# yuliangguo/OmniFusion

Measured on AMD Instinct MI355X. Metric: panoramas/sec at 512x1024 ERP, N=18 256^2 patches; equi2pers+pers2equi GB/s vs HBM peak, higher is better.
Workload: dtype f16x3 (fp16 hi/lo pairs, fp32 accumulate: fp32-class); 1 GPU; cfg2/cfg4 shard: 8 panoramas/GPU/step, 512x1024 ERP, fov 80, nrows 4 (18 patches); full single-pass spherical_fusion forward (confidence=True) at patch size 128 — the only size the reference network exists at (SURVEY 0.1); random-init weights (seed 42); inputs resident in HBM; resample pair at 18x256^2 reported in roofline_resample; per_gpu_batch=8, global_batch=8, parallelism=image-sharded x1, execution=3 forwards in flight per GPU on 3 streams (spherical_fusion.pipelined)

## Files before the change

### include/omnifusion.h

```cpp
#ifndef OMNIFUSION_H_
#define OMNIFUSION_H_

#include <stddef.h>
#include <stdint.h>

#ifdef __cplusplus
extern "C" {
#endif

#define OMNI_VERSION 200

enum omni_status {
    OMNI_OK = 0,
    OMNI_ERR_INVALID = 1,
    OMNI_ERR_HIP = 2,
    OMNI_ERR_UNSUPPORTED = 3
};

enum omni_layout { OMNI_LAYOUT_BCHWN = 0, OMNI_LAYOUT_BNCHW = 1, OMNI_LAYOUT_BNHWC = 2,
                   OMNI_LAYOUT_BCHNW = 3  };
enum omni_dtype { OMNI_F32 = 0, OMNI_F16 = 1 };

typedef void* omni_stream_t;
typedef struct omni_geometry omni_geometry_t;
// ... 40 lines not shown

int omni_equi2pers_bwd(const void* grad_pers, void* grad_erp, int dtype, int B, int C, int H, int W,
                       int ph, int pw, int nrows, float fov_h, float fov_w, int layout, omni_stream_t stream);
int omni_pers2equi_bwd(const void* grad_erp, void* grad_pers, int dtype, int B, int C, int ph, int pw,
                       int H, int W, int nrows, float fov_h, float fov_w, int layout, omni_stream_t stream);
int omni_conv2d_nhwc_f32(const float* src1, const float* src2, const float* wt, const float* bias,
                         const float* res, float* dst, int M, int H, int W, int C1, int C2, int Cout,
                         int KH, int KW, int stride, int pad, int act, omni_stream_t stream);
int omni_conv2d_splitk_plan(long long rows, int Cout, int ksteps);
int omni_conv2d_nhwc_f32_ws(const float* src1, const float* src2, const float* wt, const float* bias,
                            const float* res, float* dst, int M, int H, int W, int C1, int C2, int Cout,
                            int KH, int KW, int stride, int pad, int act, int splitk, float* ws, size_t ws_bytes,
                            omni_stream_t stream);
int omni_conv2d_nhwc_f16x3_ws(const float* src1, const float* src2, const void* wt16, const float* bias,
                              const float* res, float* dst, int M, int H, int W, int C1, int C2, int Cout,
                              int KH, int KW, int stride, int pad, int act, int splitk, float* ws, size_t ws_bytes,
                              omni_stream_t stream);
int omni_conv2d_sh_f16x3_ws(const void* src1, const void* src2, const void* wt16, const float* bias,
                            const void* res, void* dst, int fmt, int M, int H, int W, int C1, int C2, int Cout,
                            int KH, int KW, int stride, int pad, int act, int splitk, float* ws, size_t ws_bytes,
                            omni_stream_t stream);
int omni_gemm_rows_sh_f16x3(const void* x, const void* wt16r, const float* bias, const float* res, void* dst, int fmt,
                            int rows, int K, int N, int act, omni_stream_t stream);
int omni_gemm_rows_pack(const void* wt16, void* wt16r, int N, int K, omni_stream_t stream);
int omni_gemm_rows_ln_sh_f16x3(const float* x, const float* ln_weight, const float* ln_bias, float eps, const void* wt16r, const float* bias,
                               const float* res, void* dst, int fmt, int rows, int N, int act, omni_stream_t stream);
int omni_conv3x3_up2_sh_f16x3(const void* src, const void* wt16, const float* bias, void* dst, int fmt,
                              int M, int Hl, int Wl, int C, int Cout, int act, omni_stream_t stream);
size_t omni_up2_heads_scratch_bytes(int M, int P);
int omni_conv3x3_up2_heads_sh_f16x3(const void* src, const void* wt16, const float* bias, const void* heads_w16f, float bias_pred, float bias_weight,
                                    float* scratch, size_t scratch_bytes, float* out_a, float* out_c, int M, int P, int confidence, omni_stream_t stream);
int omni_conv3x3_up2_heads_sh_f16x1(const void* src, const void* wt16, const float* bias, const void* heads_w16f, float bias_pred, float bias_weight,
                                    float* scratch, size_t scratch_bytes, float* out_a, float* out_c, int M, int P, int confidence, omni_stream_t stream);
int omni_heads_pack_f16x3(const float* w_host, void* dst_host);
int omni_conv2d_sh_f16x3_post_ws(const void* src1, const void* src2, const void* wt16, const float* bias,
                                 const void* res, void* dst, int fmt, int M, int H, int W, int C1, int C2, int Cout,
                                 int KH, int KW, int stride, int pad, int act, int splitk, float* ws, size_t ws_bytes,
                                 const float* post, size_t post_elems, omni_stream_t stream);
int omni_wino_input_sh(const void* src, void* V, int M, int H, int W, int C, omni_stream_t stream);
int omni_conv3x3_wino_sh_f16x3(const void* V, const void* wt16, const float* bias, const void* res, void* dst, int fmt,
                               int M, int H, int W, int C, int Cout, int act, int splitk, float* ws, size_t ws_bytes, omni_stream_t stream);
int omni_sh_from_f32(const float* src, void* dst, size_t n, omni_stream_t stream);
int omni_sh_to_f32(const void* src, float* dst, size_t n, omni_stream_t stream);
int omni_sh_overflow(int* flag, int reset);
int omni_stem_f32(const float* src, const float* wt, const float* bias, float* dst, int M, int P, omni_stream_t stream);
int omni_maxpool3x3s2_f32(const float* src, float* dst, int M, int H, int W, int C, omni_stream_t stream);
int omni_upsample_bilinear_f32(const float* src, float* dst, int M, int H, int W, int C, int Ho, int Wo, omni_stream_t stream);
int omni_add_hw_f32(float* x, const float* y, int M, int HW, int C, omni_stream_t stream);
int omni_add_period_f32(float* x, const float* y, size_t total, size_t period, omni_stream_t stream);
int omni_stem_sh(const float* src, const float* wt, const float* bias, void* dst, int M, int P, omni_stream_t stream);
int omni_stem_sh_f16x3(const float* src, const void* wt16, const float* bias, void* dst, int M, int P, omni_stream_t stream);
int omni_stem_sh_f16x1(const float* src, const void* wt16, const float* bias, void* dst, int M, int P, omni_stream_t stream);
int omni_maxpool3x3s2_sh(const void* src, void* dst, int M, int H, int W, int C, omni_stream_t stream);
int omni_upsample_bilinear_sh(const void* src, void* dst, int M, int H, int W, int C, int Ho, int Wo, omni_stream_t stream);
int omni_up2_tapsum_sh(const float* y, const float* bias, void* dst, int M, int Hl, int Wl, int Cout, int act, omni_stream_t stream);
int omni_add_hw_sh(void* x, const float* y, int M, int HW, int C, omni_stream_t stream);
int omni_add_period_sh(void* x, const float* y, size_t total, size_t period, omni_stream_t stream);
int omni_layernorm512_sh(const float* x, const float* g, const float* b, void* y, int rows, float eps, omni_stream_t stream);
int omni_gemm_rows_slices_sh_f16x3(const void* x, const void* wt16r, float* parts, int rows, int K, int N, int slices, omni_stream_t stream);
int omni_gemm_rows_ln_parts_sh_f16x3(const float* parts, int nparts, const float* pbias, const float* pres, float* xout,
                                     const float* ln_weight, const float* ln_bias, float eps, const void* wt16r, const float* bias,
                                     void* dst, int fmt, int rows, int N, int act, omni_stream_t stream);
int omni_splitk_reduce_ln512(const float* parts, int nparts, const float* bias, const float* res, float* tok, const float* ln_weight, const float* ln_bias,
                             float eps, void* y, int fmt, int rows, omni_stream_t stream);
int omni_gemm_sh_f16x3_ln512_ws(const void* x, const void* wt16, const float* bias, const float* res, float* tok, const float* ln_g, const float* ln_b,
                                float eps, void* y, int fmt, int rows, int K, int splitk, float* ws, size_t ws_bytes, omni_stream_t stream);
int omni_attention_qkv_sh(const float* qkv, void* out, int B, int N, omni_stream_t stream);
int omni_token_pack_f32(const float* d, const float* pos, float* tok, int M, int N, int HW, int C, omni_stream_t stream);
int omni_layernorm512_f32(const float* x, const float* g, const float* b, float* y, int rows, float eps, omni_stream_t stream);
int omni_attention_f32(const float* q, const float* kv, float* out, int B, int N, omni_stream_t stream);
int omni_heads_f32(const float* x, const float* w, float bias_pred, float bias_weight, float* out_a, float* out_c,
                   int M, int P, int confidence, omni_stream_t stream);
int omni_mlp_points_f32(const float* xyz, const float* depth, const float* w1, const float* b1, const float* w2,
                        const float* b2, float* out, int Mo, int N, int HW, omni_stream_t stream);

int omni_masked_median_f32(const float* x, const float* mask, size_t n, unsigned* ws, float* out, omni_stream_t stream);
int omni_depth_metrics_f32(float* pred, const float* gt, const float* mask, const float* scale_num, const float* scale_den,
                           size_t n, double* ws, float* out, omni_stream_t stream);

size_t omni_semantic_workspace_bytes(size_t npix);
int omni_semantic_step_f32(const float* logits, const int64_t* target, int B, int C, size_t HW, int64_t ignore_index, int K,
                           void* workspace, float* loss, int64_t* pred, int64_t* confusion, omni_stream_t stream);
int omni_semantic_grad_f32(const float* logits, const int64_t* target, int B, int C, size_t HW, int64_t ignore_index,
                           const void* workspace, const float* grad_out, float* grad_logits, omni_stream_t stream);
int omni_confusion_matrix_i64(const int64_t* pred, const int64_t* gt, size_t n, int K, int64_t* confusion, int64_t* n_bad,
                              omni_stream_t stream);

int omni_preprocess_rgb_u8(const unsigned char* src_hwc, float* dst_chw, int B, int Hs, int Ws, int H, int W, omni_stream_t stream);
int omni_preprocess_depth_u16(const unsigned short* src, float* depth, unsigned char* mask, int B, int Hs, int Ws, int H, int W,
                              float min_depth, float max_depth, omni_stream_t stream);
int omni_png_info(const void* data, size_t nbytes, int* width, int* height, int* bit_depth, int* color_type);
int omni_png_decode(const void* data, size_t nbytes, void* dst, int H, int W, int kind);
int omni_png_decode_batch(const void* const* datas, const size_t* nbytes, void* const* dsts, int n, int H, int W, int kind, int threads);
int omni_zlib_inflate(const void* src, size_t nbytes, void* dst, size_t cap, size_t* produced, size_t* consumed);
int omni_png_checksums(const void* data, size_t nbytes, unsigned* crc32, unsigned* adler32);
size_t omni_berhu_workspace_bytes(int B);
int omni_berhu_loss_f32(const float* pred, const float* gt, const float* mask, const float* weights, int B, size_t per_item,
                        void* workspace, float* loss, omni_stream_t stream);
int omni_berhu_grad_f32(const float* pred, const float* gt, const float* mask, const float* weights, int B, size_t per_item,
                        const void* workspace, const float* grad_out, float* grad_pred, omni_stream_t stream);
int omni_pointcloud_ply_f32(const float* depth, const float* rgb, unsigned char* records, int B, int H, int W, omni_stream_t stream);

size_t omni_dibr_workspace_bytes(int B, int C, int H, int W);
int omni_splat_render_f32(const float* img, const float* depth, const float* coords, float max_depth,
                          float* recon, unsigned char* mask , int B, int C, int H, int W,
                          void* workspace, omni_stream_t stream);
// ... 85 lines not shown
```

### omnifusion_amd/_lib.py

```python
import ctypes
import os

_HERE = os.path.dirname(os.path.abspath(__file__))
LIB_PATH = os.environ.get("OMNI_LIB_VARIANT") or os.path.join(_HERE, "csrc", "libomnifusion_hip.so")
LIB_PATH_DEBUG = os.path.join(_HERE, "csrc", "libomnifusion_hip_dbg.so")

OMNI_OK, OMNI_ERR_INVALID, OMNI_ERR_HIP, OMNI_ERR_UNSUPPORTED = 0, 1, 2, 3
LAYOUT_BCHWN, LAYOUT_BNCHW, LAYOUT_BNHWC, LAYOUT_BCHNW = 0, 1, 2, 3
F32, F16 = 0, 1

_lib = None


class OmniLibraryMissing(ImportError):
    pass


EXPORTS = [
    "omni_version", "omni_last_error", "omni_set_option", "omni_get_option", "omni_num_patches", "omni_patch_centers",
    "omni_geometry_create", "omni_geometry_destroy", "omni_geometry_cache_clear", "omni_geometry_cache_size",
    "omni_equi2pers", "omni_equi2pers_aux", "omni_pers2equi", "omni_pers2equi_conf", "omni_patches_to_planar",
    "omni_equi2pers_g", "omni_pers2equi_g", "omni_equi2pers_bwd", "omni_pers2equi_bwd",
    "omni_conv2d_nhwc_f32", "omni_stem_f32", "omni_maxpool3x3s2_f32", "omni_upsample_bilinear_f32",
    "omni_add_hw_f32", "omni_add_period_f32", "omni_token_pack_f32", "omni_layernorm512_f32",
    "omni_attention_f32", "omni_heads_f32", "omni_mlp_points_f32",
    "omni_conv2d_nhwc_f16x3_ws", "omni_conv2d_sh_f16x3_ws", "omni_conv2d_sh_f16x3_post_ws", "omni_gemm_rows_sh_f16x3", "omni_gemm_rows_ln_sh_f16x3", "omni_gemm_rows_pack", "omni_conv3x3_up2_sh_f16x3", "omni_conv3x3_up2_heads_sh_f16x3", "omni_conv3x3_up2_heads_sh_f16x1", "omni_up2_heads_scratch_bytes", "omni_heads_pack_f16x3", "omni_sh_from_f32", "omni_sh_to_f32", "omni_sh_overflow",
    "omni_stem_sh", "omni_stem_sh_f16x3", "omni_stem_sh_f16x1", "omni_maxpool3x3s2_sh", "omni_upsample_bilinear_sh", "omni_up2_tapsum_sh", "omni_add_hw_sh", "omni_add_period_sh", "omni_layernorm512_sh", "omni_gemm_sh_f16x3_ln512_ws", "omni_gemm_rows_slices_sh_f16x3", "omni_gemm_rows_ln_parts_sh_f16x3", "omni_splitk_reduce_ln512", "omni_wino_input_sh", "omni_conv3x3_wino_sh_f16x3", "omni_attention_qkv_sh",
    "omni_conv2d_splitk_plan", "omni_conv2d_nhwc_f32_ws",
    "omni_masked_median_f32", "omni_depth_metrics_f32",
    "omni_png_info", "omni_png_decode", "omni_png_decode_batch", "omni_zlib_inflate", "omni_png_checksums",
    "omni_preprocess_rgb_u8", "omni_preprocess_depth_u16", "omni_berhu_workspace_bytes", "omni_berhu_loss_f32", "omni_berhu_grad_f32",
    "omni_pointcloud_ply_f32",
    "omni_dibr_workspace_bytes", "omni_splat_render_f32", "omni_dibr_f32",
    "omni_splat_render_wt_f32", "omni_dibr_wt_f32", "omni_dibr_bwd_workspace_bytes", "omni_splat_render_bwd_f32", "omni_dibr_bwd_f32",
    "omni_ssim_f32", "omni_photometric_workspace_bytes", "omni_photometric_grad_scratch_bytes", "omni_photometric_loss_f32",
    "omni_photometric_grad_f32",
    "omni_freeview_rotations", "omni_freeview_equi2pers_f32", "omni_freeview_pers2equi_f32", "omni_freeview_merge_f32",
    "omni_freeview_bwd_workspace_bytes", "omni_freeview_equi2pers_bwd_f32", "omni_freeview_pers2equi_bwd_f32", "omni_freeview_merge_bwd_f32",
    "omni_semantic_workspace_bytes", "omni_semantic_step_f32", "omni_semantic_grad_f32", "omni_confusion_matrix_i64",
    "omni_depth_normals_f32", "omni_sobel_f32", "omni_l1_workspace_bytes", "omni_l1_loss_f32", "omni_l1_grad_f32",
    "omni_geometry_terms_workspace_bytes", "omni_geometry_terms_f32", "omni_geometry_terms_grad_f32",
    "omni_image_diff_f32", "omni_image_diff_norm_f32", "omni_vertex_diff_norm_f32",
    "omni_guided_smoothness_workspace_bytes", "omni_guided_smoothness_f32", "omni_guided_smoothness_grad_f32",
    "omni_depth_smoothness_workspace_bytes", "omni_depth_smoothness_f32", "omni_depth_smoothness_grad_f32",
    "omni_chamfer_workspace_bytes", "omni_chamfer_nn_f32", "omni_chamfer_grad_f32",
]


def load():
    global _lib
    if _lib is not None:
        return _lib
    if not os.path.exists(LIB_PATH):
        raise OmniLibraryMissing(
            f"{LIB_PATH} not found: build it with `python -m omnifusion_amd.build` "
            "(hipcc --offload-arch=gfx950).  There is no fallback path.")
    import torch
    lib = ctypes.CDLL(LIB_PATH)
    lib.omni_last_error.restype = ctypes.c_char_p
    lib.omni_version.restype = ctypes.c_int
    lib.omni_up2_heads_scratch_bytes.restype = ctypes.c_size_t
    lib.omni_dibr_workspace_bytes.restype = ctypes.c_size_t
    lib.omni_splat_render_f32.argtypes = [ctypes.c_void_p] * 3 + [ctypes.c_float] + [ctypes.c_void_p] * 2 + [ctypes.c_int] * 4 + [ctypes.c_void_p] * 2
    lib.omni_dibr_f32.argtypes = [ctypes.c_void_p] * 4 + [ctypes.c_int, ctypes.c_float, ctypes.c_int] + [ctypes.c_void_p] * 2 + \
        [ctypes.c_int] * 4 + [ctypes.c_void_p] * 2
    vp, ci, cf = ctypes.c_void_p, ctypes.c_int, ctypes.c_float
    lib.omni_splat_render_wt_f32.argtypes = [vp] * 3 + [cf] + [vp] * 3 + [ci] * 4 + [vp] * 2
    lib.omni_dibr_wt_f32.argtypes = [vp] * 4 + [ci, cf, ci] + [vp] * 3 + [ci] * 4 + [vp] * 2
    lib.omni_dibr_bwd_workspace_bytes.restype = ctypes.c_size_t
    lib.omni_splat_render_bwd_f32.argtypes = [vp] * 6 + [cf] + [vp] * 3 + [ci] * 4 + [vp] * 2
    lib.omni_dibr_bwd_f32.argtypes = [vp] * 7 + [ci, cf, ci] + [vp] * 2 + [ci] * 4 + [vp] * 2
    lib.omni_ssim_f32.argtypes = [vp] * 2 + [ci] * 5 + [vp, ci, vp, vp]
    lib.omni_photometric_workspace_bytes.restype = ctypes.c_size_t
    lib.omni_photometric_grad_scratch_bytes.restype = ctypes.c_size_t
    lib.omni_photometric_loss_f32.argtypes = [vp, vp, vp, ci, vp, ci] + [ci] * 5 + [vp, ci, cf] + [vp] * 3
    lib.omni_photometric_grad_f32.argtypes = [vp, vp, vp, ci, vp, ci] + [ci] * 5 + [vp, ci, cf] + [vp] * 5
    lib.omni_freeview_rotations.argtypes = [vp, vp, ci, vp, vp]
    lib.omni_freeview_equi2pers_f32.argtypes = [vp] * 3 + [ci] * 7 + [cf, cf, ci, vp]
    lib.omni_freeview_pers2equi_f32.argtypes = [vp] * 4 + [ci] * 6 + [cf, cf, vp]
    lib.omni_freeview_merge_f32.argtypes = [vp] * 4 + [ci] * 7 + [cf, cf, vp]
# ... 94 lines not shown
```

### omnifusion_amd/csrc/omni_net.hip

```cpp
#include <algorithm>
#include "omni_internal.h"
#include "omni_sh.h"

namespace {
typedef float f4v __attribute__((ext_vector_type(4)));

template <bool SH>
__global__ __launch_bounds__(256) void stem_kernel(const float* __restrict__ src, const float* __restrict__ wt,
                                                   const float* __restrict__ bias, void* __restrict__ dst,
                                                   int M, int P, int Po)
{
    __shared__ __attribute__((aligned(16))) float wl[147 * 64];
    __shared__ float in[3][21][22];
    const int t = threadIdx.x;
    const int tiles = Po / 8;
    const int m = blockIdx.x / (tiles * tiles), tt = blockIdx.x % (tiles * tiles);
    const int oy0 = (tt / tiles) * 8, ox0 = (tt % tiles) * 8;
    for (int i = t; i < 147 * 64 / 4; i += 256) reinterpret_cast<f4v*>(wl)[i] = reinterpret_cast<const f4v*>(wt)[i];
    const int iy0 = oy0 * 2 - 3, ix0 = ox0 * 2 - 3;
    for (int i = t; i < 3 * 21 * 21; i += 256) {
        const int c = i / 441, r = (i % 441) / 21, q = i % 21;
        const int iy = iy0 + r, ix = ix0 + q;
        float v = 0.0f;
        if ((unsigned)iy < (unsigned)P && (unsigned)ix < (unsigned)P) v = src[((size_t)m * 3 + c) * P * P + (size_t)iy * P + ix];
// ... 335 lines not shown
            for (int kx = 0; kx < 3; ++kx) {
                const float* px = tile + ((ly + ky) * (HT + 2) + lx + kx) * HPITCH;
                const float* w0 = w + (ky * 3 + kx) * 32; const float* w1 = w0 + 288;
#pragma unroll
                for (int c = 0; c < 32; c += 4) {
                    const f4v v = *reinterpret_cast<const f4v*>(px + c);
                    ap = fmaf(v.x, w0[c], ap); ap = fmaf(v.y, w0[c + 1], ap); ap = fmaf(v.z, w0[c + 2], ap); ap = fmaf(v.w, w0[c + 3], ap);
                    aw = fmaf(v.x, w1[c], aw); aw = fmaf(v.y, w1[c + 1], aw); aw = fmaf(v.z, w1[c + 2], aw); aw = fmaf(v.w, w1[c + 3], aw);
                }
            }
        const int m = tid / (tiles * tiles), tt = tid % (tiles * tiles);
        const int oy = (tt / tiles) * HT + ly, ox = (tt % tiles) * HT + lx;
        if (oy < P && ox < P) {
            const size_t i = ((size_t)m * P + oy) * P + ox;
            const float pr = fmaxf(ap, 0.0f), cf = 1.0f / (1.0f + expf(-aw));
            outa[i] = conf ? pr * cf : pr;
            if (outc) outc[i] = cf;
        }
    }
}

__global__ __launch_bounds__(256) void mlp_points_kernel(const float* __restrict__ xyz, const float* __restrict__ depth,
                                                         const float* __restrict__ w1 , const float* __restrict__ b1,
                                                         const float* __restrict__ w2 , const float* __restrict__ b2,
                                                         float* __restrict__ out, int Mo, int N, int HW)
{
    const int i = blockIdx.x * 256 + threadIdx.x;
    if (i >= Mo * HW) return;
    const int m = i / HW, hw = i % HW, n = m % N;
    const float d = depth ? depth[i] : 1.0f;
    const float x0 = xyz[((size_t)n * 3 + 0) * HW + hw] * d, x1 = xyz[((size_t)n * 3 + 1) * HW + hw] * d, x2 = xyz[((size_t)n * 3 + 2) * HW + hw] * d;
    float hid[16];
#pragma unroll
    for (int j = 0; j < 16; ++j) hid[j] = fmaxf(fmaf(x2, w1[j * 3 + 2], fmaf(x1, w1[j * 3 + 1], fmaf(x0, w1[j * 3], b1[j]))), 0.0f);
    float* o = out + (size_t)i * 64;
    for (int j = 0; j < 64; j += 4) {
        float r[4];
#pragma unroll
        for (int e = 0; e < 4; ++e) {
            float acc = b2[j + e];
#pragma unroll
            for (int k = 0; k < 16; ++k) acc = fmaf(hid[k], w2[(j + e) * 16 + k], acc);
            r[e] = fmaxf(acc, 0.0f);
        }
        f4v v; v.x = r[0]; v.y = r[1]; v.z = r[2]; v.w = r[3];
        *reinterpret_cast<f4v*>(o + j) = v;
    }
}

inline int nblk(size_t n) { return (int)((n + 255) / 256); }
}

#define S_ (hipStream_t)stream
OMNI_SH_OVERFLOW_ACCESSOR(omni_sh_overflow_net)

extern "C" {

int omni_stem_f32(const float* src, const float* wt, const float* bias, float* dst, int M, int P, omni_stream_t stream)
{
    if (P % 16) OMNI_FAIL(OMNI_ERR_INVALID, "omni_stem: patch size must be a multiple of 16");
    const int Po = P / 2;
    hipLaunchKernelGGL(stem_kernel<false>, dim3(M * (Po / 8) * (Po / 8)), dim3(256), 0, S_, src, wt, bias, (void*)dst, M, P, Po);
    OMNI_HIP(hipGetLastError()); return OMNI_OK;
}
int omni_maxpool3x3s2_f32(const float* src, float* dst, int M, int H, int W, int C, omni_stream_t stream)
{
    const int Ho = (H + 2 - 3) / 2 + 1, Wo = (W + 2 - 3) / 2 + 1;
    hipLaunchKernelGGL(maxpool_kernel<false>, dim3(nblk((size_t)M * Ho * Wo * C / 4)), dim3(256), 0, S_, (const void*)src, (void*)dst, M, H, W, C, Ho, Wo);
    OMNI_HIP(hipGetLastError()); return OMNI_OK;
}
int omni_upsample_bilinear_f32(const float* src, float* dst, int M, int H, int W, int C, int Ho, int Wo, omni_stream_t stream)
{
    hipLaunchKernelGGL(upsample_kernel<false>, dim3(nblk((size_t)M * Ho * Wo * C / 4)), dim3(256), 0, S_, (const void*)src, (void*)dst, M, H, W, C, Ho, Wo,
                       (float)H / (float)Ho, (float)W / (float)Wo);
    OMNI_HIP(hipGetLastError()); return OMNI_OK;
}
int omni_add_hw_f32(float* x, const float* y, int M, int HW, int C, omni_stream_t stream)
{
    const size_t total = (size_t)M * HW * C;
    hipLaunchKernelGGL(add_hw_kernel, dim3(nblk(total)), dim3(256), 0, S_, x, y, total, HW, C);
    OMNI_HIP(hipGetLastError()); return OMNI_OK;
}
int omni_add_period_f32(float* x, const float* y, size_t total, size_t period, omni_stream_t stream)
{
    hipLaunchKernelGGL(add_period_kernel, dim3(nblk(total)), dim3(256), 0, S_, x, y, total, period);
    OMNI_HIP(hipGetLastError()); return OMNI_OK;
}
int omni_stem_sh(const float* src, const float* wt, const float* bias, void* dst, int M, int P, omni_stream_t stream)
{
    if (P % 16) OMNI_FAIL(OMNI_ERR_INVALID, "omni_stem: patch size must be a multiple of 16");
    const int Po = P / 2;
    hipLaunchKernelGGL(stem_kernel<true>, dim3(M * (Po / 8) * (Po / 8)), dim3(256), 0, S_, src, wt, bias, dst, M, P, Po);
    OMNI_HIP(hipGetLastError()); return OMNI_OK;
}
int omni_maxpool3x3s2_sh(const void* src, void* dst, int M, int H, int W, int C, omni_stream_t stream)
{
    if (C % 32) OMNI_FAIL(OMNI_ERR_INVALID, "SH tensors need C % 32 == 0");
    const int Ho = (H + 2 - 3) / 2 + 1, Wo = (W + 2 - 3) / 2 + 1;
    hipLaunchKernelGGL(maxpool_kernel<true>, dim3(nblk((size_t)M * Ho * Wo * C / 4)), dim3(256), 0, S_, src, dst, M, H, W, C, Ho, Wo);
    OMNI_HIP(hipGetLastError()); return OMNI_OK;
}
int omni_upsample_bilinear_sh(const void* src, void* dst, int M, int H, int W, int C, int Ho, int Wo, omni_stream_t stream)
{
    if (C % 32) OMNI_FAIL(OMNI_ERR_INVALID, "SH tensors need C % 32 == 0");
    hipLaunchKernelGGL(upsample_sh8_kernel, dim3(nblk((size_t)M * Ho * Wo * C / 8)), dim3(256), 0, S_, (const unsigned char*)src,
                       (unsigned char*)dst, M, H, W, C, Ho, Wo, (float)H / (float)Ho, (float)W / (float)Wo);
    OMNI_HIP(hipGetLastError()); return OMNI_OK;
// ... 78 lines not shown
```

### omnifusion_amd/isa.py

```python
import os
import re
import subprocess
import sys
import tempfile

LLVM = os.environ.get("OMNI_LLVM_BIN", "/opt/rocm/lib/llvm/bin")
TARGET = "hipv4-amdgcn-amd-amdhsa--gfx950"
FORBIDDEN = re.compile(r"\bv_pk_(mul|add|fma)_f32\b")
COUNTED = ("e2p_box_kernel", "p2e_lds_kernel", "p2e_walk_kernel", "e2p_ref_kernel")
HOT = ("conv_sh_kernel", "conv3x3_halo_sh_kernel", "conv3x3_up2_g1_kernel", "stem_f16x3_pc_kernel", "heads_kernel", "maxpool_kernel",
       "layernorm512_kernel", "attention_kernel", "upsample_sh8_kernel")
HOST_ONLY = ("omni_png.o", "omni_geometry.o")


def _device_object(obj, tmp):
    fat = os.path.join(tmp, "fat.bin")
    co = os.path.join(tmp, "dev.co")
    r = subprocess.run([os.path.join(LLVM, "llvm-objcopy"), "--dump-section", f".hip_fatbin={fat}", obj, os.path.join(tmp, "copy.o")],
                       stderr=subprocess.DEVNULL)
    if r.returncode != 0 or not os.path.exists(fat) or os.path.getsize(fat) == 0:
        return None
    subprocess.check_call([os.path.join(LLVM, "clang-offload-bundler"), "--unbundle", "--type=o", f"--input={fat}",
                           f"--targets={TARGET}", f"--output={co}"])
    return co


def disassemble(obj):
    with tempfile.TemporaryDirectory() as tmp:
        co = _device_object(obj, tmp)
        if co is None:
            return ""
        return subprocess.check_output([os.path.join(LLVM, "llvm-objdump"), "-d", "--mcpu=gfx950", co]).decode()


def kernel_meta(obj):
    with tempfile.TemporaryDirectory() as tmp:
        co = _device_object(obj, tmp)
        if co is None:
            return []
        txt = subprocess.check_output([os.path.join(LLVM, "llvm-readelf"), "--notes", co]).decode()
    out, cur = [], None
    keys = {".vgpr_count": "vgpr", ".agpr_count": "agpr", ".sgpr_count": "sgpr", ".group_segment_fixed_size": "lds",
            ".private_segment_fixed_size": "scratch", ".vgpr_spill_count": "vgpr_spill", ".sgpr_spill_count": "sgpr_spill",
            ".name": "name"}
    for line in txt.splitlines():
        m = re.match(r"^  - \.(\w+):\s*(\S+)\s*$", line)
        if m:
            cur = {}
            out.append(cur)
            line = "    ." + m.group(1) + ": " + m.group(2)
        m = re.match(r"^    (\.\w+):\s*(\S+)\s*$", line)
        if m and cur is not None and m.group(1) in keys:
            v = m.group(2)
            cur[keys[m.group(1)]] = v if m.group(1) == ".name" else int(v)
    return [k for k in out if "name" in k]


def demangle(names):
    try:
        p = subprocess.run([os.path.join(LLVM, "llvm-cxxfilt")], input="\n".join(names).encode(), stdout=subprocess.PIPE, check=True)
        return p.stdout.decode().splitlines()
    except Exception:
        return list(names)
# ... 69 lines not shown
```

### omnifusion_amd/model/_engine.py

```python
import ctypes
import os

import torch

from .. import _lib
from ..equi_pers.equi2pers_v3 import equi2pers_patches, equi2pers_aux, pair, _NPATCH
from ..equi_pers.pers2equi_v3 import pers2equi, pers2equi_conf

ACT_NONE, ACT_RELU, ACT_GELU = 0, 1, 2
_LAYERS = [("layer1", 3, 1), ("layer2", 4, 2), ("layer3", 6, 2), ("layer4", 3, 2)]
_BN_EPS = 1e-5
PRECISIONS = ("f16x3", "f16x1", "fp32")


def _p(t):
    return ctypes.c_void_p(t.data_ptr()) if t is not None else None


def split_weights_f16x3(w):
    w = w.to(torch.float32)
    wmax = float(w.abs().max()) if w.numel() else 0.0
    if not wmax < 65504.0:
        raise ValueError(f"folded weight magnitude {wmax:g} is outside the fp16 range of the f16x3 operand format: "
                         "run this checkpoint with OMNI_NET_PRECISION=fp32")
# ... 314 lines not shown
        pending = None
        for i in range(6):
            t = f"t{i}."
            if sh:
                if pending is not None:
                    tok, qkv = self._ln_gemm_parts(pending, t + "norm1.weight", t + "norm1.bias", 1e-5, t + "attn.qkv.w16", M, 1536)
                    pending = None
                elif normed is not None:
                    qkv = self._gemm_sh(normed, t + "attn.qkv.w16", None, M, 512, 1536)
                else:
                    qkv = self._ln_gemm_sh(tok, t + "norm1.weight", t + "norm1.bias", 1e-5, t + "attn.qkv.w16", None, M, 1536)
                att = new(M, 512)
                _lib.check(lib.omni_attention_qkv_sh(_p(qkv), _p(att), bs, N, self._s), "attention")
                tok = self._gemm_sh(att, t + "attn.proj.w16", t + "attn.proj.bias", M, 512, 512, res=tok)
                h = self._ln_gemm_sh(tok, t + "norm2.weight", t + "norm2.bias", 1e-5, t + "mlp.fc1.w16", t + "mlp.fc1.bias", M, 2048, act=ACT_GELU, out_sh=True)
                nxt = (f"t{i + 1}.norm1.weight", f"t{i + 1}.norm1.bias", 1e-5, True) if i < 5 else ("enc_norm.w", "enc_norm.b", 1e-6, False)
                tok, normed, pending = self._fc2_ln(h, t + "mlp.fc2.w16", t + "mlp.fc2.bias", M, tok, nxt)
                continue
            y = self._ln(tok, t + "norm1.weight", t + "norm1.bias", M, 1e-5)
            q = self._gemm(y, t + "attn.q.weight", None, M, 512, 512)
            kv = self._gemm(y, t + "attn.kv.weight", None, M, 512, 1024)
            att = new(M, 512)
            _lib.check(lib.omni_attention_f32(_p(q), _p(kv), _p(att), bs, N, self._s), "attention")
            tok = self._gemm(att, t + "attn.proj.weight", t + "attn.proj.bias", M, 512, 512, res=tok)
            y = self._ln(tok, t + "norm2.weight", t + "norm2.bias", M, 1e-5)
            h = self._gemm(y, t + "mlp.fc1.weight", t + "mlp.fc1.bias", M, 512, 2048, act=ACT_GELU)
            tok = self._gemm(h, t + "mlp.fc2.weight", t + "mlp.fc2.bias", M, 2048, 512, res=tok)
        if sh and pending is not None:
            parts, S, bkey, res_tok = pending
            tok_sum, tok = new(M, 512), new(M, 512)
            _lib.check(lib.omni_splitk_reduce_ln512(_p(parts), S, _p(self.w[bkey]), _p(res_tok), _p(tok_sum), _p(self.w["enc_norm.w"]), _p(self.w["enc_norm.b"]),
                                                    ctypes.c_float(1e-6), _p(tok), 0, M, self._s), "reduce+ln")
        else:
            tok = normed if (sh and normed is not None) else self._ln(tok, "enc_norm.w", "enc_norm.b", M, 1e-6)
        return tok

    def network(self, patches, point_feat, bs, confidence, out=None):
        lib = _lib.load()
        dev = patches.device
        self._s = ctypes.c_void_p(torch.cuda.current_stream(dev).cuda_stream)
        N, P = self.npatches, self.patch_size[0]
        M = bs * N
        self._bs = bs
        P2, P4, P8, P16, P32 = P // 2, P // 4, P // 8, P // 16, P // 32
        new = lambda *s: torch.empty(s, dtype=torch.float32, device=dev)
        conv1 = new(M, P2, P2, 64)
        sh = self.sh
        x = new(M, P4, P4, 64)
        pat = patches.view(M, 3, P, P)
        for m0, m1 in self._chunks(bs, N, self.front_chunk):
            Mc = m1 - m0
            if self.terms == 1 and P % 32:
                raise ValueError(f"precision f16x1 needs a patch size that is a multiple of 32 (got {P})")
            if sh and P % 32 == 0:
                _lib.check((lib.omni_stem_sh_f16x1 if self._x1 else lib.omni_stem_sh_f16x3)(_p(pat[m0:m1]), _p(self.w["stem.w16"]), _p(self.w["stem.b"]), _p(conv1[m0:m1]), Mc, P, self._s), "stem")
            else:
                _lib.check((lib.omni_stem_sh if sh else lib.omni_stem_f32)(_p(pat[m0:m1]), _p(self.w["stem.w"]), _p(self.w["stem.b"]),
                                                                            _p(conv1[m0:m1]), Mc, P, self._s), "stem")
            _lib.check((lib.omni_maxpool3x3s2_sh if sh else lib.omni_maxpool3x3s2_f32)(_p(conv1[m0:m1]), _p(x[m0:m1]), Mc, P2, P2, 64, self._s), "maxpool")
        feats = {}
        cin, size = 64, P4
        for lname, nblk, stride in _LAYERS:
            cout = {"layer1": 64, "layer2": 128, "layer3": 256, "layer4": 512}[lname]
            for i in range(nblk):
                p = f"{lname}.{i}"
                s = stride if i == 0 else 1
                ident = x
                if (p + ".ds.w") in self.w:
                    ident = self._conv(x, p + ".ds", M, size, size, cin, cout, 1, s, 0, ACT_NONE)
                y = self._conv(x, p + ".c1", M, size, size, cin, cout, 3, s, 1, ACT_RELU)
                size = (size + 2 - 3) // s + 1
                fold = sh and self.fold_point_feat and lname == "layer1" and i == nblk - 1
                x = self._conv(y, p + ".c2", M, size, size, cout, cout, 3, 1, 1, ACT_RELU, res=ident, post=point_feat if fold else None)
                cin = cout
            if lname == "layer1" and not (sh and self.fold_point_feat):
                _lib.check((lib.omni_add_period_sh if sh else lib.omni_add_period_f32)(
                    _p(x), _p(point_feat), ctypes.c_size_t(x.numel()), ctypes.c_size_t(point_feat.numel()), self._s), "add point_feat")
            feats[lname] = x
        layer1, layer2, layer3, layer4 = (feats[k] for k in ("layer1", "layer2", "layer3", "layer4"))
        if 32 * P32 * P32 != 512:
            raise RuntimeError(f"patch size {P}: token dim {32 * P32 * P32} != 512 — the reference network only exists at "
                               "patch size 128 (SURVEY.md finding 0.1)")
        d = self._conv(layer4, "down", M, P32, P32, 512, 32, 1, 1, 0, ACT_NONE, out_f32=True)
        tok = self.transformer(d, bs)
        _lib.check((lib.omni_add_hw_sh if sh else lib.omni_add_hw_f32)(_p(layer4), _p(tok), M, P32 * P32, 512, self._s), "token bias")
        x = self._up_conv_taps(layer4, "de_conv0_0", M, P32, P32, 512, 256, ACT_RELU)
        x = self._conv(x, "de_conv0_1", M, P16, P16, 256, 128, 3, 1, 1, ACT_RELU, x2=layer3, C2=256)
        x = self._up_conv_taps(x, "de_conv1_0", M, P16, P16, 128, 128, ACT_RELU)
        x = self._conv(x, "de_conv1_1", M, P8, P8, 128, 64, 3, 1, 1, ACT_RELU, x2=layer2, C2=128)
        x = self._up_conv(x, "de_conv2_0", M, P8, P8, 64, 64, ACT_RELU)
        x = self._conv(x, "de_conv2_1", M, P4, P4, 64, 64, 3, 1, 1, ACT_RELU, x2=layer1, C2=64)
        a, c = out if out is not None else (new(bs, N, 1, P, P), new(bs, N, 1, P, P) if confidence else None)
        av, cv = a.view(M, P, P), c.view(M, P, P) if c is not None else None
        fused = sh and self.fuse_heads and P % 32 == 0
        x_in, de4 = x, (None if fused else new(M, P, P, 32))
        for m0, m1 in self._chunks(bs, N, self.tail_chunk):
            Mc = m1 - m0
            x = self._up_conv(x_in[m0:m1], "de_conv3_0", Mc, P4, P4, 64, 64, ACT_RELU)
            x = self._conv(x, "de_conv3_1", Mc, P2, P2, 64, 32, 3, 1, 1, ACT_RELU, x2=conv1[m0:m1], C2=64)
            if fused:
                nb = int(lib.omni_up2_heads_scratch_bytes(Mc, P))
                hs = new((nb + 3) // 4)
                _lib.check((lib.omni_conv3x3_up2_heads_sh_f16x1 if self._x1 else lib.omni_conv3x3_up2_heads_sh_f16x3)(_p(x), _p(self.w["de_conv4_0.w16"]), _p(self.w["de_conv4_0.b"]), _p(self.w["heads.w16f"]),
                                                               ctypes.c_float(self.head_bias[0]), ctypes.c_float(self.head_bias[1]), _p(hs), ctypes.c_size_t(nb),
                                                               _p(av[m0:m1]), _p(cv[m0:m1]) if cv is not None else None, Mc, P, 1 if confidence else 0, self._s), "up+conv+heads")
                continue
            self._up_conv(x, "de_conv4_0", Mc, P2, P2, 32, 32, ACT_RELU, out_f32=True, out=de4[m0:m1])
            _lib.check(lib.omni_heads_f32(_p(de4[m0:m1]), _p(self.w["heads.w"]), ctypes.c_float(self.head_bias[0]), ctypes.c_float(self.head_bias[1]),
                                          _p(av[m0:m1]), _p(cv[m0:m1]) if cv is not None else None, Mc, P, 1 if confidence else 0, self._s), "heads")
        self.last = {"de_conv4_0": de4, "layer4": layer4}
        return a, c

    fuse_heads = os.environ.get("OMNI_FUSE_HEADS", "1") != "0"

    tail_chunk = 0
    front_chunk = 0

    @staticmethod
    def _chunks(bs, N, per):
        per = bs if per <= 0 else min(per, bs)
        return [(b0 * N, min(bs, b0 + per) * N) for b0 in range(0, bs, per)]

    def blend(self, a, c, erp_hw):
        P = self.patch_size
        if c is not None:
            return pers2equi_conf(a, c, self.fov, self.nrows, P, erp_hw, layout=_lib.LAYOUT_BNCHW)
        return pers2equi(a, self.fov, self.nrows, P, erp_hw, None, layout=_lib.LAYOUT_BNCHW)

    def mlp_points(self, name, xyz, depth, Mo):
        lib = _lib.load()
        P4 = self.patch_size[0] // 4
        out = torch.empty((Mo, P4, P4, 64), dtype=torch.float32, device=xyz.device)
        s = ctypes.c_void_p(torch.cuda.current_stream(xyz.device).cuda_stream)
        _lib.check(lib.omni_mlp_points_f32(_p(xyz), _p(depth), _p(self.w[name + ".w1"]), _p(self.w[name + ".b1"]),
                                           _p(self.w[name + ".w2"]), _p(self.w[name + ".b2"]), _p(out), Mo, self.npatches,
                                           P4 * P4, s), "mlp_points")
        return out

    def check_input(self, rgb):
        if not isinstance(rgb, torch.Tensor) or rgb.dim() != 4 or rgb.shape[1] != 3:
            raise ValueError("expected an RGB panorama batch [B,3,H,W]")
        if not rgb.is_cuda:
            raise ValueError("the model runs on an MI355X only (got a CPU tensor); there is no CPU path")
        if rgb.dtype != torch.float32:
            raise ValueError("float32 input expected")
        if _NPATCH[self.nrows] != self.npatches:
            raise ValueError("npatches does not match nrows")
```

Before: 4149 panoramas/s.

## Fuse ResNet stem conv with 3x3 stride-2 maxpool in one warp-specialized kernel

Adds a kernel that computes the 7x7 stride-2 stem conv on an output tile plus a one-pixel halo using MFMA f16x3. It keeps the tile in LDS and applies the 3x3/s2 maxpool there, writing both conv1 and the pooled output. Producer waves prefetch and split the input image into double-buffered LDS while consumer waves compute, which hides load latency. This removes the separate maxpool launch and its reread of conv1 from HBM. The cost is recomputing halo pixels per tile and a complex kernel with high LDS use, which may limit occupancy.

```diff
diff --git a/include/omnifusion.h b/include/omnifusion.h
--- a/include/omnifusion.h
+++ b/include/omnifusion.h
@@ -116,6 +116,7 @@
 int omni_stem_sh_f16x3(const float* src, const void* wt16, const float* bias, void* dst, int M, int P, omni_stream_t stream);
 int omni_stem_sh_f16x1(const float* src, const void* wt16, const float* bias, void* dst, int M, int P, omni_stream_t stream);
 int omni_maxpool3x3s2_sh(const void* src, void* dst, int M, int H, int W, int C, omni_stream_t stream);
+int omni_stem_pool_sh_f16x3(const float* src, const void* wt16, const float* bias, void* conv1, void* pooled, int M, int P, omni_stream_t stream);
 int omni_upsample_bilinear_sh(const void* src, void* dst, int M, int H, int W, int C, int Ho, int Wo, omni_stream_t stream);
 int omni_up2_tapsum_sh(const float* y, const float* bias, void* dst, int M, int Hl, int Wl, int Cout, int act, omni_stream_t stream);
 int omni_add_hw_sh(void* x, const float* y, int M, int HW, int C, omni_stream_t stream);
diff --git a/omnifusion_amd/_lib.py b/omnifusion_amd/_lib.py
--- a/omnifusion_amd/_lib.py
+++ b/omnifusion_amd/_lib.py
@@ -25,7 +25,7 @@
     "omni_add_hw_f32", "omni_add_period_f32", "omni_token_pack_f32", "omni_layernorm512_f32",
     "omni_attention_f32", "omni_heads_f32", "omni_mlp_points_f32",
     "omni_conv2d_nhwc_f16x3_ws", "omni_conv2d_sh_f16x3_ws", "omni_conv2d_sh_f16x3_post_ws", "omni_gemm_rows_sh_f16x3", "omni_gemm_rows_ln_sh_f16x3", "omni_gemm_rows_pack", "omni_conv3x3_up2_sh_f16x3", "omni_conv3x3_up2_heads_sh_f16x3", "omni_conv3x3_up2_heads_sh_f16x1", "omni_up2_heads_scratch_bytes", "omni_heads_pack_f16x3", "omni_sh_from_f32", "omni_sh_to_f32", "omni_sh_overflow",
-    "omni_stem_sh", "omni_stem_sh_f16x3", "omni_stem_sh_f16x1", "omni_maxpool3x3s2_sh", "omni_upsample_bilinear_sh", "omni_up2_tapsum_sh", "omni_add_hw_sh", "omni_add_period_sh", "omni_layernorm512_sh", "omni_gemm_sh_f16x3_ln512_ws", "omni_gemm_rows_slices_sh_f16x3", "omni_gemm_rows_ln_parts_sh_f16x3", "omni_splitk_reduce_ln512", "omni_wino_input_sh", "omni_conv3x3_wino_sh_f16x3", "omni_attention_qkv_sh",
+    "omni_stem_sh", "omni_stem_sh_f16x3", "omni_stem_sh_f16x1", "omni_maxpool3x3s2_sh", "omni_stem_pool_sh_f16x3", "omni_upsample_bilinear_sh", "omni_up2_tapsum_sh", "omni_add_hw_sh", "omni_add_period_sh", "omni_layernorm512_sh", "omni_gemm_sh_f16x3_ln512_ws", "omni_gemm_rows_slices_sh_f16x3", "omni_gemm_rows_ln_parts_sh_f16x3", "omni_splitk_reduce_ln512", "omni_wino_input_sh", "omni_conv3x3_wino_sh_f16x3", "omni_attention_qkv_sh",
     "omni_conv2d_splitk_plan", "omni_conv2d_nhwc_f32_ws",
     "omni_masked_median_f32", "omni_depth_metrics_f32",
     "omni_png_info", "omni_png_decode", "omni_png_decode_batch", "omni_zlib_inflate", "omni_png_checksums",
diff --git a/omnifusion_amd/csrc/omni_net.hip b/omnifusion_amd/csrc/omni_net.hip
--- a/omnifusion_amd/csrc/omni_net.hip
+++ b/omnifusion_amd/csrc/omni_net.hip
@@ -411,7 +411,13 @@
 }
 
 #define S_ (hipStream_t)stream
-OMNI_SH_OVERFLOW_ACCESSOR(omni_sh_overflow_net)
+OMNI_SH_OVERFLOW_ACCESSOR(omni_sh_overflow_net_own)
+int omni_sh_overflow_stem_pool(unsigned* out, int reset);
+int omni_sh_overflow_net(unsigned* out, int reset)
+{
+    const int a = omni_sh_overflow_net_own(out, reset), b = omni_sh_overflow_stem_pool(out, reset);
+    return (a != 0 || b != 0) ? -1 : 0;
+}
 
 extern "C" {
 
diff --git a/omnifusion_amd/csrc/omni_stem_pool.hip b/omnifusion_amd/csrc/omni_stem_pool.hip
--- /dev/null
+++ b/omnifusion_amd/csrc/omni_stem_pool.hip
@@ -0,0 +1,252 @@
+#include "omni_conv_sh_common.h"
+
+namespace {
+
+constexpr int SP_TH = 8, SP_TW = 16;
+constexpr int SP_WH = SP_TH + 1, SP_WW = SP_TW + 1, SP_NPIX = SP_WH * SP_WW;
+constexpr int SP_IH = 2 * SP_WH + 5, SP_IW = 2 * SP_WW + 5, SP_IP = 40, SP_IS = 48;
+constexpr int SP_G = 6;
+constexpr int SP_IMG = 3 * SP_IH * SP_IP, SP_IPT = (SP_IMG + 255) / 256, SP_IMGS = 3 * SP_IH * SP_IS;
+constexpr int SP_PITCH = 272;
+constexpr int SP_NBLK = (SP_NPIX + 31) / 32;
+constexpr int SP_CONS = 2 * SP_NBLK;
+constexpr int SP_THREADS = 64 * (SP_CONS + 4);
+constexpr int SP_COPY = SP_TH * SP_TW * 16 / 64;
+constexpr int SP_POOL = (SP_TH / 2) * (SP_TW / 2) * 8 / 64;
+static_assert(SP_IW + 1 <= SP_IP && SP_IP <= SP_IS, "the kx = 7 slot of the last window column reads a parked zero");
+
+__global__ __launch_bounds__(SP_THREADS) void stem_pool_sh_kernel(const float* __restrict__ src, const void* __restrict__ wt16, const float* __restrict__ bias,
+                                                                  void* __restrict__ conv1, void* __restrict__ pooled, int M, int P, int tpb)
+{
+    __shared__ __attribute__((aligned(1024))) unsigned char wl[64 * SP_G * 128];
+    __shared__ __attribute__((aligned(16))) _Float16 imh[2][SP_IMGS], iml[2][SP_IMGS];
+    __shared__ __attribute__((aligned(16))) unsigned char otile[2][SP_NPIX * SP_PITCH];
+    __shared__ __attribute__((aligned(16))) float sbias[64];
+    const int t = threadIdx.x, lane = t & 63;
+    const int wave = __builtin_amdgcn_readfirstlane(t >> 6);
+    const int Po = P / 2, Pq = P / 4;
+    const int sps = Po / SP_TH, tps = Po / SP_TW, ntiles = M * sps * tps;
+    const int T0 = blockIdx.x * tpb, T1 = min(T0 + tpb, ntiles);
+    if (T0 >= T1) return;
+    auto where = [&](int T, int& m, int& oy0, int& ox0) { const int strip = T / tps; ox0 = (T - strip * tps) * SP_TW; m = strip / sps; oy0 = (strip - m * sps) * SP_TH; };
+
+    if (wave >= SP_CONS) {
+        const int ft = t - 64 * SP_CONS;
+        float pre[SP_IPT], nxt[SP_IPT];
+        int po[SP_IPT], rq[SP_IPT], ls[SP_IPT];
+#pragma unroll
+        for (int k = 0; k < SP_IPT; ++k) {
+            const int i = ft + 256 * k;
+            const int c = i / (SP_IH * SP_IP), r = (i % (SP_IH * SP_IP)) / SP_IP, q = i % SP_IP;
+            po[k] = (c * P + r) * P + q;
+            rq[k] = (i < SP_IMG && q < SP_IW) ? (r | (q << 8)) : -1;
+            ls[k] = i < SP_IMG ? (i / SP_IP) * SP_IS + q : -1;
+        }
+        int fm, fs, fc;
+        { const int strip = T0 / tps; fc = T0 - strip * tps; fm = strip / sps; fs = strip - fm * sps; }
+        auto fetch = [&](float (&v)[SP_IPT]) {
+            const int m = fm, oy0 = fs * SP_TH, ox0 = fc * SP_TW;
+            if (++fc == tps) { fc = 0; if (++fs == sps) { fs = 0; ++fm; } }
+            const int iy0 = oy0 * 2 - 5, ix0 = ox0 * 2 - 5;
+            const float* base = src + (size_t)m * 3 * P * P + ((long long)iy0 * P + ix0);
+#pragma unroll
+            for (int k = 0; k < SP_IPT; ++k) {
+                const int iy = iy0 + (rq[k] & 0xff), ix = ix0 + (rq[k] >> 8);
+                v[k] = (rq[k] >= 0 && (unsigned)iy < (unsigned)P && (unsigned)ix < (unsigned)P) ? base[po[k]] : 0.0f;
+            }
+        };
+        auto park = [&](int b, const float (&v)[SP_IPT]) {
+#pragma unroll
+            for (int k = 0; k < SP_IPT; ++k) {
+                const float x = v[k];
+                const _Float16 hh = (fabsf(x) < 6.103515625e-05f) ? (_Float16)0.0f : (_Float16)x;
+                if (ls[k] >= 0) { imh[b][ls[k]] = hh; iml[b][ls[k]] = (_Float16)((x - (float)hh) * 2048.0f); }
+            }
+        };
+        fetch(pre);
+        if (T0 + 1 < T1) fetch(nxt);
+        park(0, pre);
+        if (T0 + 2 < T1) fetch(pre);
+        __syncthreads();
+        int b = 0, T = T0 + 1;
+        for (;;) {
+            if (T >= T1) break;
+            b ^= 1; park(b, nxt);
+            if (T + 2 < T1) fetch(nxt);
+            __syncthreads();
+            if (++T >= T1) break;
+            b ^= 1; park(b, pre);
+            if (T + 2 < T1) fetch(pre);
+            __syncthreads();
+            ++T;
+        }
+        __syncthreads();
+        return;
+    }
+
+    const int blk = wave % SP_NBLK, cj = wave / SP_NBLK;
+    if (wave < 8) {
+        const int pr = wave & 3, ch = wave >> 2;
+        const int gs = (lane & 15) ^ ((4 * pr + (lane >> 4)) & 15);
+        const int rl = 8 * pr + 2 * (lane >> 4) + (gs >> 3), pc16 = (gs & 7) * 16;
+        const rsrc_t rsw = make_rsrc(wt16, (size_t)64 * SP_G * 128);
+#pragma unroll
+        for (int g = 0; g < SP_G; ++g)
+            dma16(rsw, wl + g * 8192 + pr * 1024 + ch * 4096, ((rl + 32 * ch) * SP_G + g) * 128 + pc16, 0);
+    }
+    int fo[4];
+    {
+        const int r = lane & 31, v = r >> 1, h = lane >> 5;
+#pragma unroll
+        for (int k = 0; k < 4; ++k) fo[k] = v * 256 + ((((r & 1) * 8 + 2 * k + h) ^ v) * 16);
+    }
+    const int npix = 32 * blk + (lane & 31);
+    const bool live = npix < SP_NPIX;
+    const int py = (live ? npix : SP_NPIX - 1) / SP_WW, px = (live ? npix : SP_NPIX - 1) % SP_WW;
+    int rowoff[2 * SP_G];
+#pragma unroll
+    for (int f = 0; f < 2 * SP_G; ++f) {
+        int rr = 2 * f + (lane >> 5);
+        rr = rr < 21 ? rr : 20;
+        rowoff[f] = ((rr / 7) * SP_IH + rr % 7 + 2 * py) * SP_IS + 2 * px;
+    }
+    if (wave == 0) sbias[lane] = bias ? bias[lane] : 0.0f;
+    wait_vm<0>();
+    wait_lds_reads();
+    __syncthreads();
+
+    f16v acc, acc1;
+    auto kloop = [&](int b) {
+        const _Float16* ih = imh[b];
+        const _Float16* il = iml[b];
+        acc = (f16v)(0.0f); acc1 = (f16v)(0.0f);
+#pragma unroll
+        for (int g = 0; g < SP_G; ++g)
+#pragma unroll
+            for (int kc = 0; kc < 2; ++kc) {
+                const int ro = rowoff[2 * g + kc];
+                h8v ah, al;
+#pragma unroll
+                for (int u = 0; u < 4; ++u) {
+                    const h2v xh = *reinterpret_cast<const h2v*>(ih + ro + 2 * u);
+                    ah[2 * u] = xh[0]; ah[2 * u + 1] = xh[1];
+                    const h2v xl = *reinterpret_cast<const h2v*>(il + ro + 2 * u);
+                    al[2 * u] = xl[0]; al[2 * u + 1] = xl[1];
+                }
+                const unsigned char* bp = wl + g * 8192 + cj * 4096;
+                const h8v bh = *reinterpret_cast<const h8v*>(bp + fo[kc]);
+                const h8v bl = *reinterpret_cast<const h8v*>(bp + fo[2 + kc]);
+                acc = __builtin_amdgcn_mfma_f32_32x32x16_f16(bh, ah, acc, 0, 0, 0);
+                acc1 = __builtin_amdgcn_mfma_f32_32x32x16_f16(bl, ah, acc1, 0, 0, 0);
+                acc1 = __builtin_amdgcn_mfma_f32_32x32x16_f16(bh, al, acc1, 0, 0, 0);
+            }
+    };
+    auto deposit = [&](int T, int ob) {
+        int m, oy0, ox0;
+        where(T, m, oy0, ox0);
+        const bool inimg = (py > 0 || oy0 > 0) && (px > 0 || ox0 > 0);
+        unsigned char* dp = otile[ob] + npix * SP_PITCH + cj * 128 + 8 * (lane >> 5);
+#pragma unroll
+        for (int q = 0; q < 4; ++q) {
+            f4v v;
+#pragma unroll
+            for (int e = 0; e < 4; ++e) v[e] = acc_join<false>(acc1[4 * q + e], acc[4 * q + e]);
+            v += *reinterpret_cast<const f4v*>(sbias + 32 * cj + 8 * q + 4 * (lane >> 5));
+#pragma unroll
+            for (int e = 0; e < 4; ++e) v[e] = inimg ? fmaxf(v[e], 0.f) : 0.0f;
+            h4v hi, lo;
+            sh_split4(v, hi, lo);
+            if (live) { *reinterpret_cast<h4v*>(dp + 16 * q) = hi; *reinterpret_cast<h4v*>(dp + 16 * q + 64) = lo; }
+        }
+    };
+    const bool pools = (wave & 2) != 0 && wave < 8;
+    static_assert(SP_COPY == 32 && SP_POOL == 4 && SP_CONS == 10, "the task split above is written for these counts");
+    auto out = [&](int T, int ob) {
+        int m, oy0, ox0;
+        where(T, m, oy0, ox0);
+        const unsigned char* tp = otile[ob];
+        auto piece = [&](int task, const unsigned char*& lp, size_t& go) {
+            const int idx = task * 64 + lane, op = idx >> 4, pc = idx & 15;
+            const int oy = op / SP_TW, ox = op % SP_TW;
+            lp = tp + ((oy + 1) * SP_WW + ox + 1) * SP_PITCH + 16 * pc;
+            go = (((size_t)m * Po + oy0 + oy) * Po + ox0 + ox) * 256 + 16 * pc;
+        };
+        {
+            const unsigned char *l0, *l1, *l2; size_t g0, g1, g2;
+            piece(wave, l0, g0); piece(wave + SP_CONS, l1, g1); piece(wave + 2 * SP_CONS, l2, g2);
+            const uint4 v0 = *reinterpret_cast<const uint4*>(l0), v1 = *reinterpret_cast<const uint4*>(l1), v2 = *reinterpret_cast<const uint4*>(l2);
+            *reinterpret_cast<uint4*>((unsigned char*)conv1 + g0) = v0;
+            *reinterpret_cast<uint4*>((unsigned char*)conv1 + g1) = v1;
+            *reinterpret_cast<uint4*>((unsigned char*)conv1 + g2) = v2;
+        }
+        if (wave < SP_COPY - 3 * SP_CONS) {
+            const unsigned char* lp; size_t go;
+            piece(3 * SP_CONS + wave, lp, go);
+            *reinterpret_cast<uint4*>((unsigned char*)conv1 + go) = *reinterpret_cast<const uint4*>(lp);
+        }
+        if (pools) {
+            const int ppy = (wave >> 2) * 2 + (wave & 1), ppx = lane >> 3, pc = lane & 7;
+            const int po8 = (pc >> 2) * 128 + (pc & 3) * 16;
+            f4v b0 = (f4v)(-INFINITY), b1 = (f4v)(-INFINITY);
+#pragma unroll
+            for (int ky = 0; ky < 3; ++ky)
+#pragma unroll
+                for (int kx = 0; kx < 3; ++kx) {
+                    const int wy = 2 * ppy + ky, wx = 2 * ppx + kx;
+                    const unsigned char* p = tp + (wy * SP_WW + wx) * SP_PITCH + po8;
+                    const h8v hi = *reinterpret_cast<const h8v*>(p), lo = *reinterpret_cast<const h8v*>(p + 64);
+                    if ((wy > 0 || oy0 > 0) && (wx > 0 || ox0 > 0)) {
+#pragma unroll
+                        for (int e = 0; e < 4; ++e) {
+                            b0[e] = fmaxf(b0[e], fmaf((float)lo[e], 4.8828125e-4f, (float)hi[e]));
+                            b1[e] = fmaxf(b1[e], fmaf((float)lo[4 + e], 4.8828125e-4f, (float)hi[4 + e]));
+                        }
+                    }
+                }
+            h4v h0, l0, h1, l1;
+            sh_split4(b0, h0, l0); sh_split4(b1, h1, l1);
+            h8v oh, ol;
+#pragma unroll
+            for (int e = 0; e < 4; ++e) { oh[e] = h0[e]; oh[4 + e] = h1[e]; ol[e] = l0[e]; ol[4 + e] = l1[e]; }
+            unsigned char* dp = (unsigned char*)pooled + (((size_t)m * Pq + oy0 / 2 + ppy) * Pq + ox0 / 2 + ppx) * 256 + po8;
+            *reinterpret_cast<h8v*>(dp) = oh;
+            *reinterpret_cast<h8v*>(dp + 64) = ol;
+        }
+    };
+    for (int T = T0; T < T1; ++T) {
+        const int b = (T - T0) & 1;
+        if (cj == 0) {
+            if (T > T0) out(T - 1, b ^ 1);
+            kloop(b);
+            deposit(T, b);
+        } else {
+            kloop(b);
+            deposit(T, b);
+            if (T > T0) out(T - 1, b ^ 1);
+        }
+        wait_lds_reads();
+        __syncthreads();
+    }
+    out(T1 - 1, (T1 - 1 - T0) & 1);
+}
+
+}
+
+OMNI_SH_OVERFLOW_ACCESSOR(omni_sh_overflow_stem_pool)
+
+extern "C" int omni_stem_pool_sh_f16x3(const float* src, const void* wt16, const float* bias, void* conv1, void* pooled, int M, int P, omni_stream_t stream)
+{
+    if (!src || !wt16 || !conv1 || !pooled) OMNI_FAIL(OMNI_ERR_INVALID, "omni_stem_pool_sh_f16x3: null pointer");
+    if (P % 32 || P <= 0 || M <= 0) OMNI_FAIL(OMNI_ERR_INVALID, "omni_stem_pool_sh_f16x3: patch size must be a multiple of 32");
+    const int Po = P / 2;
+    const long long strips = (long long)M * (Po / SP_TH), tps = Po / SP_TW, nt = strips * tps;
+    if (nt > 0x7fffffffLL) OMNI_FAIL(OMNI_ERR_INVALID, "omni_stem_pool_sh_f16x3: too many tiles");
+    const int ntiles = (int)nt;
+    const int split = (strips < 256 && Po % (4 * SP_TW) == 0) ? 4 : (strips < 512 && Po % (2 * SP_TW) == 0) ? 2 : 1;
+    int tpb = (int)tps / split;
+    const int ncu = omni_num_cus();
+    if (split == 1 && ntiles > ncu * tps) tpb = (ntiles + ncu - 1) / ncu;
+    hipLaunchKernelGGL(stem_pool_sh_kernel, dim3((unsigned)((ntiles + tpb - 1) / tpb)), dim3(SP_THREADS), 0, (hipStream_t)stream, src, wt16, bias, conv1, pooled, M, P, tpb);
+    OMNI_HIP(hipGetLastError());
+    return OMNI_OK;
+}
diff --git a/omnifusion_amd/isa.py b/omnifusion_amd/isa.py
--- a/omnifusion_amd/isa.py
+++ b/omnifusion_amd/isa.py
@@ -8,7 +8,7 @@
 TARGET = "hipv4-amdgcn-amd-amdhsa--gfx950"
 FORBIDDEN = re.compile(r"\bv_pk_(mul|add|fma)_f32\b")
 COUNTED = ("e2p_box_kernel", "p2e_lds_kernel", "p2e_walk_kernel", "e2p_ref_kernel")
-HOT = ("conv_sh_kernel", "conv3x3_halo_sh_kernel", "conv3x3_up2_g1_kernel", "stem_f16x3_pc_kernel", "heads_kernel", "maxpool_kernel",
+HOT = ("conv_sh_kernel", "conv3x3_halo_sh_kernel", "conv3x3_up2_g1_kernel", "stem_f16x3_pc_kernel", "stem_pool_sh_kernel", "heads_kernel", "maxpool_kernel",
        "layernorm512_kernel", "attention_kernel", "upsample_sh8_kernel")
 HOST_ONLY = ("omni_png.o", "omni_geometry.o")
 
diff --git a/omnifusion_amd/model/_engine.py b/omnifusion_amd/model/_engine.py
--- a/omnifusion_amd/model/_engine.py
+++ b/omnifusion_amd/model/_engine.py
@@ -390,6 +390,9 @@
             Mc = m1 - m0
             if self.terms == 1 and P % 32:
                 raise ValueError(f"precision f16x1 needs a patch size that is a multiple of 32 (got {P})")
+            if self.fuse_pool and self.terms == 3 and P % 32 == 0:
+                _lib.check(lib.omni_stem_pool_sh_f16x3(_p(pat[m0:m1]), _p(self.w["stem.w16"]), _p(self.w["stem.b"]), _p(conv1[m0:m1]), _p(x[m0:m1]), Mc, P, self._s), "stem+maxpool")
+                continue
             if sh and P % 32 == 0:
                 _lib.check((lib.omni_stem_sh_f16x1 if self._x1 else lib.omni_stem_sh_f16x3)(_p(pat[m0:m1]), _p(self.w["stem.w16"]), _p(self.w["stem.b"]), _p(conv1[m0:m1]), Mc, P, self._s), "stem")
             else:
@@ -454,6 +457,8 @@
     tail_chunk = 0
     front_chunk = 0
 
+    fuse_pool = os.environ.get("OMNI_FUSE_POOL", "1") != "0"
+
     @staticmethod
     def _chunks(bs, N, per):
         per = bs if per <= 0 else min(per, bs)
```

New measurement: 4170 panoramas/s (median of 4 runs). Within noise of the previous version (+0.5%).
